# iSach/SoccerNeRFs

Measured on AMD Instinct MI355X. Metric: train rays/sec (K-Planes Broadcast-style, whole job), higher is better.
Workload: dtype bf16; 1 GPU; K-Planes default multiscale-res 1-16 on synthetic Broadcast-style (k-planes preset: 4096 rays/GPU/step, samples 256/128/64, 5 scales x 6 planes C=32, 156.0 M params), full train step incl. Adam; rays_per_gpu=4096, images=627, params=156049664, parallelism=single GPU

## Files before the change

### include/snerf.h

```cpp
#ifndef SNERF_H
#define SNERF_H

#include <stdint.h>

#ifdef __cplusplus
extern "C" {
#endif

typedef void* snerf_stream_t;

#define SNERF_OK 0
#define SNERF_ERR_ARG (-1)
#define SNERF_ERR_UNSUPPORTED (-2)

#define SNERF_MAX_SCALES 8
#define SNERF_ABI_VERSION 16
#define SNERF_ABI_REVISION 2

int snerf_abi_version(void);
int snerf_abi_revision(void);
const char* snerf_last_error(void);
const char* snerf_target_arch(void);

typedef struct {
// ... 177 lines not shown
  float* acc_out;
  float* depth_median;
  float* sqerr_rays;
  float* dist_rays;
  float* g_rgb;
  float* g_density;
  float* g_weights;
  int32_t* nonfinite_flag;
} snerf_ray_train_args;
int snerf_ray_train_fwd_bwd(const snerf_ray_train_args* args, snerf_stream_t stream);

int snerf_render_bwd(const float* weights, const float* rgb, const float* bg, int32_t bg_mode, const float* g_rgb_out,
                     const float* g_acc, int32_t R, int32_t S, float* g_weights, float* g_rgb, int32_t accumulate_w,
                     snerf_stream_t stream);

int snerf_render_mse_bwd(const float* weights, const float* rgb, const float* bg, int32_t bg_mode, const float* rgb_out, const float* target,
                         float go_scale, int32_t R, int32_t S, float* g_weights, float* g_rgb, float* sqerr_rays, snerf_stream_t stream);

int snerf_distortion(const float* weights, const float* sbins, int32_t R, int32_t S, float grad_scale, float* loss_rays,
                     float* g_weights, int32_t accumulate, snerf_stream_t stream);

int snerf_interlevel(const float* c_bins, const float* w_nerf, int32_t S, const float* p_bins, const float* w_prop, int32_t Sp,
                     int32_t R, float grad_scale, float* loss_rays, float* g_wprop, snerf_stream_t stream);

int snerf_depth_loss(const float* weights, const float* ebins, const float* termination_depth, const float* directions_norm, float sigma,
                     int32_t R, int32_t S, float grad_scale, float* loss_rays, float* g_weights, int32_t accumulate, snerf_stream_t stream);

int snerf_urf_depth_loss(const float* weights, const float* ebins, const float* termination_depth, const float* directions_norm,
                         const float* predicted_depth, float sigma, int32_t R, int32_t S, float grad_scale, float* loss_rays, float* g_weights,
                         float* g_predicted_depth, int32_t accumulate, snerf_stream_t stream);


int snerf_plane_reg(const snerf_kplanes_desc* desc, const float* planes, float* grad, float c_space_tv, float c_time_smooth,
                    float c_sparse, float* losses, int32_t n_slots, int32_t overwrite, snerf_stream_t stream);

typedef struct {
  int32_t nonfinite;
  int32_t t;
  int32_t skipped;
  int32_t dropped;
  float step_size;
  float inv_sqrt_bc2;
  int32_t skip;
  int32_t _pad;
} snerf_adam_dyn;
int snerf_adam_prepare(snerf_adam_dyn* dyn, float lr, float beta1, float beta2, int32_t policy, int32_t force_nonfinite, snerf_stream_t stream);
// ... 352 lines not shown
```

### soccernerfs_amd/_lib.py

```python
import ctypes as C
import os

import torch

_PKG = os.path.dirname(os.path.abspath(__file__))
LIB_PATH = os.path.join(_PKG, "libsnerf.so")

MAX_SCALES = 8
ABI_VERSION = 16
ABI_REVISION = 2


class KPlanesDesc(C.Structure):
    _c_struct_ = "snerf_kplanes_desc"
    _fields_ = [
        ("n_scales", C.c_int32),
        ("C", C.c_int32),
        ("concat", C.c_int32),
        ("n_coords", C.c_int32),
        ("res", (C.c_int32 * 4) * MAX_SCALES),
        ("off", (C.c_int64 * 6) * MAX_SCALES),
    ]


# ... 38 lines not shown
                ("gdens", C.c_void_p), ("grad_planes", C.c_void_p), ("workspace", C.c_void_p), ("gX", C.c_void_p)]


class AdamDyn(C.Structure):
    _c_struct_ = "snerf_adam_dyn"
    _fields_ = [("nonfinite", C.c_int32), ("t", C.c_int32), ("skipped", C.c_int32), ("dropped", C.c_int32),
                ("step_size", C.c_float), ("inv_sqrt_bc2", C.c_float), ("skip", C.c_int32), ("_pad", C.c_int32)]


class RenderArgs(C.Structure):
    _c_struct_ = "snerf_render_args"
    _fields_ = [("weights", C.c_void_p), ("rgb", C.c_void_p), ("ebins", C.c_void_p), ("bg", C.c_void_p),
                ("R", C.c_int32), ("S", C.c_int32), ("bg_mode", C.c_int32), ("training", C.c_int32),
                ("rgb_out", C.c_void_p), ("acc_out", C.c_void_p), ("depth_median", C.c_void_p), ("depth_expected", C.c_void_p),
                ("median_rgb", C.c_void_p), ("median_index", C.c_void_p)]


class RayTrainArgs(C.Structure):
    _c_struct_ = "snerf_ray_train_args"
    _fields_ = [("density", C.c_void_p), ("ebins", C.c_void_p), ("sbins", C.c_void_p), ("rgb", C.c_void_p), ("bg", C.c_void_p), ("target", C.c_void_p),
                ("R", C.c_int32), ("S", C.c_int32), ("bg_mode", C.c_int32), ("go_scale", C.c_float), ("dist_scale", C.c_float),
                ("weights", C.c_void_p), ("rgb_out", C.c_void_p), ("acc_out", C.c_void_p), ("depth_median", C.c_void_p), ("sqerr_rays", C.c_void_p),
                ("dist_rays", C.c_void_p), ("g_rgb", C.c_void_p), ("g_density", C.c_void_p), ("g_weights", C.c_void_p), ("nonfinite_flag", C.c_void_p)]


class RaygenArgs(C.Structure):
    _c_struct_ = "snerf_raygen_args"
    _fields_ = [("indices", C.c_void_p), ("fx", C.c_void_p), ("fy", C.c_void_p), ("cx", C.c_void_p), ("cy", C.c_void_p),
                ("c2w", C.c_void_p), ("cam_times", C.c_void_p),
                ("R", C.c_int32), ("collide", C.c_int32), ("training", C.c_int32), ("near_plane", C.c_float),
                ("aabb_min", C.c_float * 3), ("aabb_max", C.c_float * 3),
                ("origins", C.c_void_p), ("dirs", C.c_void_p), ("pixel_area", C.c_void_p), ("dir_norm", C.c_void_p),
                ("times", C.c_void_p), ("nears", C.c_void_p), ("fars", C.c_void_p)]


class RaygenFrameArgs(C.Structure):
    _c_struct_ = "snerf_raygen_frame_args"
    _fields_ = [("fx", C.c_float), ("fy", C.c_float), ("cx", C.c_float), ("cy", C.c_float), ("c2w", C.c_float * 12), ("time", C.c_float),
                ("W", C.c_int32), ("H", C.c_int32), ("_pad", C.c_int32), ("p0", C.c_int64), ("p1", C.c_int64),
                ("near_plane", C.c_float), ("aabb_min", C.c_float * 3), ("aabb_max", C.c_float * 3),
                ("origins", C.c_void_p), ("dirs", C.c_void_p), ("pixel_area", C.c_void_p), ("dir_norm", C.c_void_p),
                ("times", C.c_void_p), ("nears", C.c_void_p), ("fars", C.c_void_p)]


class RaygenLensArgs(C.Structure):
    _c_struct_ = "snerf_raygen_lens_args"
# ... 81 lines not shown
    "snerf_mlp_bwd_x16_quotient": "s:PPPILPIIPPIPIPPPP",
    "snerf_mlp_bwd_fx": "s:PPPILPIIPPIPP",
    "snerf_kplanes_field_fwd_supported": "i:PPP",
    "snerf_kplanes_field_fwd": "s:PPPLPPPPPPPPPP",
    "snerf_kplanes_field_fwd_ordered": "s:PPPLPPPPPPPPPPP",
    "snerf_kplanes_field_render_supported": "i:PPPI",
    "snerf_kplanes_field_render": "s:PPPIPPPPFPPPPPPP",
    "snerf_kplanes_color_input_fwd": "s:PIPLPP",
    "snerf_kplanes_color_input_bwd": "s:PILPP",
    "snerf_kplanes_color_bwd_vd_supported": "i:P",
    "snerf_kplanes_color_bwd_vd": "s:PPPIPLPIPPP",
    "snerf_kplanes_color_bwd_vd_ws": "s:PPPIPLPIPPP",
    "snerf_kplanes_density_fwd_supported": "i:PP",
    "snerf_kplanes_density_fwd": "s:PPPLPPPPP",
    "snerf_kplanes_density_bwd_supported": "i:PP",
    "snerf_kplanes_density_bwd": "s:PIP",
    "snerf_kplanes_density_bwd_budget": "s:PIIP",
    "snerf_render_fwd": "s:PP",
    "snerf_ray_train_fwd_bwd": "s:PP",
    "snerf_render_bwd": "s:PPPIPPIIPPIP",
    "snerf_render_mse_bwd": "s:PPPIPPFIIPPPP",
    "snerf_distortion": "s:PPIIFPPIP",
    "snerf_interlevel": "s:PPIPPIIFPPP",
    "snerf_depth_loss": "s:PPPPFIIFPPIP",
    "snerf_urf_depth_loss": "s:PPPPPFIIFPPPIP",
    "snerf_plane_reg": "s:PPPFFFPIIP",
    "snerf_adam_prepare": "s:PFFFIIP",
    "snerf_adam_step": "s:PPPPPLFFFFIFIPP",
    "snerf_adam_planes_step": "s:PPPPPPFFFPIFFFFIFIPP",
    "snerf_adam_planes_step_range": "s:PPPPPPFFFPIFFFFIFILLPP",
    "snerf_comm_unique_id": "s:P",
    "snerf_comm_create": "s:IIPP",
    "snerf_comm_destroy": "s:P",
    "snerf_allreduce_grads": "s:PPLP",
    "snerf_raygen": "s:PP",
    "snerf_raygen_frame": "s:PP",
    "snerf_raygen_lens": "s:PP",
    "snerf_raygen_frame_lens": "s:PP",
    "snerf_raygen_cam": "s:PP",
    "snerf_raygen_frame_cam": "s:PP",
    "snerf_pose_apply": "s:PPPIIPP",
    "snerf_raygen_pose_bwd": "s:PP",
    "snerf_sample_pixels_uniform": "s:PIIIIPPPP",
    "snerf_sample_pixels_sphere": "s:PIIIIPPPP",
    "snerf_mask_pack": "s:PLLLPPP",
    "snerf_sample_pixels_masked": "s:PIIIIPPLPPPP",
# ... 109 lines not shown
```

### soccernerfs_amd/csrc/per_ray_common.hpp

```cpp
#pragma once
#include "common.hpp"

namespace snerf {

constexpr int RAYS_PER_BLOCK = 4;
constexpr int MAX_S = 64 * WSCAN_PER;

struct BlockSync { __device__ __forceinline__ static void sync() { __syncthreads(); } };
struct WaveSync { __device__ __forceinline__ static void sync() { wave_lds_publish(); } };

template <typename Sync>
__device__ __forceinline__ void ray_optical_depth(const float* eb, const float* sigma, int n_sigma, float* dd, float* aux, int S, int lane) {
#pragma clang fp contract(off)
  for (int i = lane; i < S; i += 64) {
    const float e0 = eb[i], e1 = eb[i + 1];
    dd[i] = (e1 - e0) * (i < n_sigma ? sigma[i] : 0.f);
  }
  Sync::sync();
  wave_scan_f64<true, false>(dd, aux, S, lane);
  Sync::sync();
}

template <typename Sync>
__device__ __forceinline__ void ray_weights(const float* eb, const float* sigma, int n_sigma, float* dd, float* aux, float* w, float* w_out, bool live,
// ... 132 lines not shown
#pragma unroll
  for (int k = 0; k < WSCAN_PER; ++k) {
    const int i = lane + 64 * k;
    if (i < S) aux[i] = gwterm[k];
  }
  Sync::sync();
  wave_scan_f64<true, true>(aux, aux, S, lane);
  Sync::sync();
#pragma unroll
  for (int k = 0; k < WSCAN_PER; ++k) {
    const int i = lane + 64 * k;
    if (i < S && live) {
      const float g = gw[i];
      const float e0 = eb[i], e1 = eb[i + 1];
      const float gdd = g * Tk[k] * ek[k] - aux[i];
      float out = gdd * (e1 - e0);
      if (!(fabsf(out) <= 3.402823466e+38f)) { out = 0.f; bad = true; }
      if (accumulate) gdens[i] += out; else gdens[i] = out;
    }
  }
  return bad;
}

}
```

### soccernerfs_amd/csrc/raygen.hip

```cpp
#include "raygen_common.hpp"

#pragma clang fp contract(off)

namespace snerf {

struct RaygenArgs {
  const int64_t* indices;
  const float* fx; const float* fy; const float* cx; const float* cy;
  const float* c2w;
  const float* cam_times;
  int R;
  float* origins; float* dirs; float* pixel_area; float* dir_norm; float* times;
  int collide; int training; float near_plane;
  float aabb_min[3], aabb_max[3];
  float* nears; float* fars;
};

__global__ void raygen_kernel(RaygenArgs a) {
  int r = blockIdx.x * blockDim.x + threadIdx.x;
  if (r >= a.R) return;
  const int64_t c = a.indices[(int64_t)r * 3], yi = a.indices[(int64_t)r * 3 + 1], xi = a.indices[(int64_t)r * 3 + 2];
  const PixelRay p = pixel_ray(yi, xi, a.fx[c], a.fy[c], a.cx[c], a.cy[c], a.c2w + c * 12);
#pragma unroll
  for (int k = 0; k < 3; ++k) { a.origins[(int64_t)r * 3 + k] = p.o[k]; a.dirs[(int64_t)r * 3 + k] = p.d[k]; }
// ... 87 lines not shown
                                                        float* __restrict__ aux_out) {
  extern __shared__ uint32_t s_w[];
  for (int i = threadIdx.x; i < n_pow2; i += blockDim.x)
    s_w[i] = i < R ? (((uint32_t)image_key[idx_in[(int64_t)i * 3]] << 14) | (uint32_t)i) : 0xffffffffu;
  __syncthreads();
  for (int k = 2; k <= n_pow2; k <<= 1)
    for (int j = k >> 1; j > 0; j >>= 1) {
      for (int t = threadIdx.x; t < n_pow2 / 2; t += blockDim.x) {
        const int i = ((t / j) * 2 * j) + (t % j), l = i + j;
        const bool up = (i & k) == 0;
        const uint32_t a = s_w[i], b = s_w[l];
        if ((a > b) == up) { s_w[i] = b; s_w[l] = a; }
      }
      __syncthreads();
    }
  for (int r = threadIdx.x; r < R; r += blockDim.x) {
    const int64_t src = s_w[r] & 0x3fffu;
#pragma unroll
    for (int c = 0; c < 3; ++c) idx_out[(int64_t)r * 3 + c] = idx_in[src * 3 + c];
    for (int c = 0; c < aux_cols; ++c) aux_out[(int64_t)r * aux_cols + c] = aux_in[src * aux_cols + c];
  }
}

__global__ __launch_bounds__(256) void ray_time_order_kernel(const float* __restrict__ times, int R, int n_pow2, int32_t* __restrict__ order_out) {
  extern __shared__ uint64_t s_tk[];
  for (int i = threadIdx.x; i < n_pow2; i += blockDim.x)
    s_tk[i] = i < R ? (((uint64_t)__float_as_uint(times[i]) << 32) | (uint32_t)i) : ~0ull;
  __syncthreads();
  for (int k = 2; k <= n_pow2; k <<= 1)
    for (int lj = 31 - __clz(k >> 1); lj >= 0; --lj) {
      const int j = 1 << lj;
      for (int t = threadIdx.x; t < n_pow2 / 2; t += blockDim.x) {
        const int i = ((t >> lj) << (lj + 1)) | (t & (j - 1)), l = i + j;
        const bool up = (i & k) == 0;
        const uint64_t a = s_tk[i], b = s_tk[l];
        if ((a > b) == up) { s_tk[i] = b; s_tk[l] = a; }
      }
      __syncthreads();
    }
  for (int r = threadIdx.x; r < R; r += blockDim.x) order_out[r] = (int32_t)(uint32_t)s_tk[r];
}

__global__ void aabb_kernel(const float* __restrict__ o, const float* __restrict__ d, int R, float near_plane, int training, const float* amin3,
                            float* __restrict__ nears, float* __restrict__ fars, float a0, float a1, float a2, float b0, float b1, float b2) {
  int r = blockIdx.x * blockDim.x + threadIdx.x;
  if (r >= R) return;
  const float mn[3] = {a0, a1, a2}, mx[3] = {b0, b1, b2};
  float tn = -INFINITY, tf = INFINITY;
#pragma unroll
  for (int k = 0; k < 3; ++k) {
    float inv = 1.f / (d[(int64_t)r * 3 + k] + 1e-6f);
    float t1 = (mn[k] - o[(int64_t)r * 3 + k]) * inv, t2 = (mx[k] - o[(int64_t)r * 3 + k]) * inv;
    tn = fmaxf(tn, fminf(t1, t2));
    tf = fminf(tf, fmaxf(t1, t2));
  }
  tn = fmaxf(tn, training ? near_plane : 0.f);
  tf = fmaxf(tf, tn + 1e-6f);
  nears[r] = tn; fars[r] = tf;
}

__global__ void pose_apply_kernel(const float* __restrict__ c2w, const float* __restrict__ adj, const int32_t* __restrict__ group, int M, int G,
                                  float* __restrict__ out) {
  const int m = blockIdx.x * blockDim.x + threadIdx.x;
// ... 199 lines not shown
  if (R == 0) return 0;
  SNERF_REQUIRE(u && indices && (!images || target), "sample_pixels_uniform: null buffer");
  hipLaunchKernelGGL(sample_pixels_kernel, dim3(ceil_div(R, 256)), dim3(256), 0, (hipStream_t)stream, u, R, M, H, W, images, indices, target);
  SNERF_LAUNCH_CHECK("sample_pixels_uniform");
  return 0;
}

extern "C" int snerf_sort_rays_by_key(const int64_t* indices_in, const int32_t* image_key, int32_t n_keys, int32_t R, const float* aux_in,
                                      int32_t aux_cols, int64_t* indices_out, float* aux_out, snerf_stream_t stream) {
  SNERF_REQUIRE(R >= 0 && R <= 16384 && n_keys >= 1 && n_keys <= (1 << 18) && aux_cols >= 0,
                "sort_rays_by_key: R=%d (<= 16384) n_keys=%d (<= 262144) aux_cols=%d", R, n_keys, aux_cols);
  if (R == 0) return 0;
  SNERF_REQUIRE(indices_in && image_key && indices_out && indices_in != indices_out && (aux_cols == 0 || (aux_in && aux_out && aux_in != aux_out)),
                "sort_rays_by_key: null or aliased buffer (the sort is out of place)");
  int n = 2;
  while (n < R) n <<= 1;
  hipLaunchKernelGGL(sort_rays_kernel, dim3(1), dim3(256), (size_t)n * sizeof(uint32_t), (hipStream_t)stream, indices_in, image_key, R, n, aux_in, aux_cols,
                     indices_out, aux_out);
  SNERF_LAUNCH_CHECK("sort_rays_by_key");
  return 0;
}

extern "C" int snerf_ray_time_order(const float* times, int32_t R, int32_t* order_out, snerf_stream_t stream) {
  SNERF_REQUIRE(R >= 0 && R <= 16384, "ray_time_order: R=%d (<= 16384: one workgroup sorts in LDS)", R);
  if (R == 0) return 0;
  SNERF_REQUIRE(times && order_out, "ray_time_order: null buffer");
  int n = 2;
  while (n < R) n <<= 1;
  SNERF_ALLOW_LDS(ray_time_order_kernel, 16384 * (int)sizeof(uint64_t));
  hipLaunchKernelGGL(ray_time_order_kernel, dim3(1), dim3(256), (size_t)n * sizeof(uint64_t), (hipStream_t)stream, times, R, n, order_out);
  SNERF_LAUNCH_CHECK("ray_time_order");
  return 0;
}

extern "C" int snerf_aabb_collide(const float* origins, const float* dirs, int32_t R, const float* aabb6, float near_plane, int32_t training,
                                  float* nears, float* fars, snerf_stream_t stream) {
  SNERF_REQUIRE(R >= 0 && aabb6, "aabb_collide: bad arguments");
  if (R == 0) return 0;
  SNERF_REQUIRE(origins && dirs && nears && fars, "aabb_collide: null buffer");
  hipLaunchKernelGGL(aabb_kernel, dim3(ceil_div(R, 256)), dim3(256), 0, (hipStream_t)stream, origins, dirs, R, near_plane, training, nullptr, nears,
                     fars, aabb6[0], aabb6[1], aabb6[2], aabb6[3], aabb6[4], aabb6[5]);
  SNERF_LAUNCH_CHECK("aabb_collide");
  return 0;
}

extern "C" int snerf_pose_apply(const float* c2w, const float* pose_adjustment, const int32_t* group, int32_t M, int32_t G, float* c2w_adj,
                                snerf_stream_t stream) {
  SNERF_REQUIRE(M >= 0 && G >= 0, "pose_apply: M=%d G=%d", M, G);
  SNERF_REQUIRE(group || G == M, "pose_apply: no group table, so G=%d must equal M=%d", G, M);
  if (M == 0) return 0;
  SNERF_REQUIRE(c2w && pose_adjustment && c2w_adj, "pose_apply: null buffer");
  hipLaunchKernelGGL(pose_apply_kernel, dim3(ceil_div(M, 256)), dim3(256), 0, (hipStream_t)stream, c2w, pose_adjustment, group, M, G, c2w_adj);
  SNERF_LAUNCH_CHECK("pose_apply");
// ... 26 lines not shown
```

### soccernerfs_amd/csrc/render_loss.hip

```cpp
#include "per_ray_common.hpp"

#pragma clang fp contract(off)

namespace snerf {

struct RenderArgs {
  const float* weights;
  const float* rgb;
  const float* ebins;
  const float* bg;
  int R, S, bg_mode, training;
  float* rgb_out;
  float* acc_out;
  float* depth_median;
  float* depth_expected;
  float* median_rgb;
  int64_t* median_index;
};

__global__ __launch_bounds__(256) void render_fwd_kernel(RenderArgs a) {
  __shared__ float s_w[RAYS_PER_BLOCK][MAX_S];
  __shared__ float s_cum[RAYS_PER_BLOCK][MAX_S];
  __shared__ int s_med[RAYS_PER_BLOCK];
  const int wv = threadIdx.x >> 6, lane = threadIdx.x & 63;
// ... 64 lines not shown
  __shared__ float s_m[RAYS_PER_BLOCK][MAX_S];
  const int wv = threadIdx.x >> 6, lane = threadIdx.x & 63;
  const int ray = blockIdx.x * RAYS_PER_BLOCK + wv;
  const bool live = ray < R;
  const int r = live ? ray : R - 1;
  for (int i = lane; i < S; i += 64) s_w[wv][i] = weights[(int64_t)r * S + i];
  const float total = ray_distortion<BlockSync>(s_w[wv], s_m[wv], sbins + (int64_t)r * (S + 1), grad_scale,
                                                g_weights && live ? g_weights + (int64_t)r * S : nullptr, accumulate != 0, S, lane);
  if (lane == 0 && live && loss_rays) loss_rays[r] = total;
}

__global__ __launch_bounds__(256) void interlevel_kernel(const float* __restrict__ c_bins, const float* __restrict__ w_nerf, int S,
                                                        const float* __restrict__ p_bins, const float* __restrict__ w_prop, int Sp, int R,
                                                        float grad_scale, float* __restrict__ loss_rays, float* __restrict__ g_wprop) {
  __shared__ float s_tp[RAYS_PER_BLOCK][MAX_S + 1];
  __shared__ float s_cy[RAYS_PER_BLOCK][MAX_S + 1];
  __shared__ float s_g[RAYS_PER_BLOCK][MAX_S];
  __shared__ int s_lo[RAYS_PER_BLOCK][MAX_S];
  __shared__ int s_hi[RAYS_PER_BLOCK][MAX_S];
  const int wv = threadIdx.x >> 6, lane = threadIdx.x & 63;
  const int ray = blockIdx.x * RAYS_PER_BLOCK + wv;
  const bool live = ray < R;
  const int r = live ? ray : R - 1;
  float* tp = s_tp[wv];
  float* cy = s_cy[wv];
  for (int i = lane; i <= Sp; i += 64) tp[i] = p_bins[(int64_t)r * (Sp + 1) + i];
  for (int i = lane; i < Sp; i += 64) cy[i + 1] = w_prop[(int64_t)r * Sp + i];
  __syncthreads();
  wave_scan_f64<false, false>(cy + 1, cy + 1, Sp, lane);
  if (lane == 0) cy[0] = 0.f;
  __syncthreads();
  float total = 0.f;
  for (int i = lane; i < S; i += 64) {
    const float c0 = c_bins[(int64_t)r * (S + 1) + i], c1 = c_bins[(int64_t)r * (S + 1) + i + 1];
    int lo = 0, hi = Sp;
    while (lo < hi) { int mid = (lo + hi) >> 1; if (tp[mid] <= c0) lo = mid + 1; else hi = mid; }
    int ilo = lo - 1; ilo = ilo < 0 ? 0 : (ilo > Sp - 1 ? Sp - 1 : ilo);
    lo = 0; hi = Sp;
    while (lo < hi) { int mid = (lo + hi) >> 1; if (tp[mid + 1] <= c1) lo = mid + 1; else hi = mid; }
    int ihi = lo; ihi = ihi < 0 ? 0 : (ihi > Sp - 1 ? Sp - 1 : ihi);
    const float wo = cy[ihi + 1] - cy[ilo];
    const float w = w_nerf[(int64_t)r * S + i];
    const float d = fmaxf(w - wo, 0.f);
    total += d * d / (w + 1.0e-7f);
    s_lo[wv][i] = ilo; s_hi[wv][i] = ihi;
    s_g[wv][i] = -2.f * d / (w + 1.0e-7f);
  }
  total = wave_sum(total);
  if (lane == 0 && live && loss_rays) loss_rays[r] = total;
  __syncthreads();
  if (g_wprop) {
    const int* slo = s_lo[wv];
    const int* shi = s_hi[wv];
    for (int j = lane; j < Sp; j += 64) {
      int a = 0, e = S;
      while (a < e) { const int mid = (a + e) >> 1; if (shi[mid] < j) a = mid + 1; else e = mid; }
      int b = 0;
      e = S;
      while (b < e) { const int mid = (b + e) >> 1; if (slo[mid] <= j) b = mid + 1; else e = mid; }
      float acc = 0.f;
      for (int i = a; i < b; ++i) acc += s_g[wv][i];
      if (live) g_wprop[(int64_t)r * Sp + j] = acc * grad_scale;
    }
  }
}

__global__ __launch_bounds__(256) void depth_loss_kernel(const float* __restrict__ weights, const float* __restrict__ ebins, const float* __restrict__ term,
                                                        const float* __restrict__ dir_norm, float sigma, int R, int S, float grad_scale,
                                                        float* __restrict__ loss_rays, float* __restrict__ g_weights, int accumulate) {
  const int wv = threadIdx.x >> 6, lane = threadIdx.x & 63;
  const int ray = blockIdx.x * RAYS_PER_BLOCK + wv;
  if (ray >= R) return;
  float D = term[ray];
  if (dir_norm) D = D * dir_norm[ray];
  const bool on = D > 0.f;
  float total = 0.f;
  for (int i = lane; i < S; i += 64) {
    const float e0 = ebins[(int64_t)ray * (S + 1) + i], e1 = ebins[(int64_t)ray * (S + 1) + i + 1];
    const float w = weights[(int64_t)ray * S + i];
    const float t = (e0 + e1) / 2.f;
    const float k = expf(-((t - D) * (t - D)) / (2.f * sigma)) * (e1 - e0);
    total += -logf(w + 1.0e-7f) * k;
    if (g_weights) {
      const float g = on ? grad_scale * (-k / (w + 1.0e-7f)) : 0.f;
      if (accumulate) g_weights[(int64_t)ray * S + i] += g; else g_weights[(int64_t)ray * S + i] = g;
    }
  }
// ... 169 lines not shown

extern "C" int snerf_distortion(const float* weights, const float* sbins, int32_t R, int32_t S, float grad_scale, float* loss_rays,
                                float* g_weights, int32_t accumulate, snerf_stream_t stream) {
  SNERF_REQUIRE(R >= 0 && S >= 1 && S <= MAX_S, "distortion: R=%d S=%d (S <= %d)", R, S, MAX_S);
  if (R == 0) return 0;
  SNERF_REQUIRE(weights && sbins, "distortion: null buffer");
  hipLaunchKernelGGL(distortion_kernel, dim3(ceil_div(R, RAYS_PER_BLOCK)), dim3(256), 0, (hipStream_t)stream, weights, sbins, R, S, grad_scale, loss_rays,
                     g_weights, accumulate);
  SNERF_LAUNCH_CHECK("distortion");
  return 0;
}

extern "C" int snerf_interlevel(const float* c_bins, const float* w_nerf, int32_t S, const float* p_bins, const float* w_prop, int32_t Sp,
                                int32_t R, float grad_scale, float* loss_rays, float* g_wprop, snerf_stream_t stream) {
  SNERF_REQUIRE(R >= 0 && S >= 1 && S <= MAX_S && Sp >= 1 && Sp <= MAX_S, "interlevel: R=%d S=%d Sp=%d", R, S, Sp);
  if (R == 0) return 0;
  SNERF_REQUIRE(c_bins && w_nerf && p_bins && w_prop, "interlevel: null buffer");
  hipLaunchKernelGGL(interlevel_kernel, dim3(ceil_div(R, RAYS_PER_BLOCK)), dim3(256), 0, (hipStream_t)stream, c_bins, w_nerf, S, p_bins, w_prop, Sp, R,
                     grad_scale, loss_rays, g_wprop);
  SNERF_LAUNCH_CHECK("interlevel");
  return 0;
}

extern "C" int snerf_ray_train_fwd_bwd(const snerf_ray_train_args* p, snerf_stream_t stream) {
  SNERF_REQUIRE(p, "ray_train_fwd_bwd: null args");
  SNERF_REQUIRE(p->R >= 0 && p->S >= 1 && p->S <= MAX_S, "ray_train_fwd_bwd: R=%d S=%d (S <= %d)", p->R, p->S, MAX_S);
  SNERF_REQUIRE(p->bg_mode == 0 || p->bg_mode == 2, "ray_train_fwd_bwd: bg_mode %d has no training backward", p->bg_mode);
  if (p->R == 0) return 0;
  SNERF_REQUIRE(p->density && p->ebins && p->sbins && p->rgb && p->bg && p->target && p->weights && p->rgb_out && p->acc_out && p->g_rgb && p->g_density,
                "ray_train_fwd_bwd: null buffer");
  RayTrainArgs a = {};
  a.density = p->density; a.ebins = p->ebins; a.sbins = p->sbins; a.rgb = p->rgb; a.bg = p->bg; a.target = p->target;
  a.R = p->R; a.S = p->S; a.bg_mode = p->bg_mode; a.go_scale = p->go_scale; a.dist_scale = p->dist_scale;
  a.weights = p->weights; a.rgb_out = p->rgb_out; a.acc_out = p->acc_out; a.depth_median = p->depth_median; a.sqerr_rays = p->sqerr_rays;
  a.dist_rays = p->dist_rays; a.g_rgb = p->g_rgb; a.g_density = p->g_density; a.g_weights = p->g_weights; a.nonfinite_flag = p->nonfinite_flag;
  hipLaunchKernelGGL(ray_train_kernel, dim3(ceil_div(p->R, RAYS_PER_BLOCK)), dim3(256), 0, (hipStream_t)stream, a);
  SNERF_LAUNCH_CHECK("ray_train_fwd_bwd");
  return 0;
}
```

### soccernerfs_amd/fused_step.py

```python
import ctypes as C
import math
from typing import Dict, Optional, Sequence, Tuple

import torch

from . import _lib


def anneal_value(step: int, max_iters: int, slope: float) -> float:
    frac = min(max(step / max_iters, 0.0), 1.0)
    return (slope * frac) / ((slope - 1) * frac + 1)


def update_schedule(step: int, warmup: int, every: int) -> float:
    return min(max(every * min(max(step / warmup, 0.0), 1.0), 1.0), float(every))


def cosine_lr_factor(step: int, warm_up_end: int, max_steps: int, alpha: float) -> float:
    if step < warm_up_end:
        return step / warm_up_end
    progress = (step - warm_up_end) / (max_steps - warm_up_end)
    return (math.cos(math.pi * progress) + 1.0) * 0.5 * (1 - alpha) + alpha


# ... 156 lines not shown
        ra.weights, ra.rgb_out, ra.acc_out = b["w"][2].data_ptr(), b["rgb_out"].data_ptr(), b["acc"].data_ptr()
        ra.depth_median = b["depth"].data_ptr() if median_depth else None
        ra.sqerr_rays, ra.dist_rays, ra.g_rgb, ra.g_density = b["sqerr"].data_ptr(), b["dist_rays"].data_ptr(), b["grgb"].data_ptr(), b["gdens"][2].data_ptr()
        ra.g_weights, ra.nonfinite_flag = None, dyn.data_ptr() if dyn is not None else None
        with self._span("ray_train_fwd_bwd"):
            self._call("ray_train_fwd_bwd", C.byref(ra), self._st)

    def _mse_distortion_bwd(self, target, bg, go_scale: float, dist_scale: float):
        b, R, S2 = self.buf, self.R, self.S[2]
        self._call("render_mse_bwd", self._p(b["w"][2]), self._p(b["rgb"]), self._p(bg), 0, self._p(b["rgb_out"]), self._p(target), go_scale, R, S2,
                   self._p(b["gw"][2]), self._p(b["grgb"]), self._p(b["sqerr"]), self._st)
        self._call("distortion", self._p(b["w"][2]), self._p(b["sb"][2]), R, S2, dist_scale, self._p(b["dist_rays"]), self._p(b["gw"][2]), 1,
                   self._st)

    def _weights_bwd(self, lvl: int, dyn: Optional[torch.Tensor] = None):
        b = self.buf
        self._call("weights_bwd", self._p(b["dens"][lvl]), self._p(b["eb"][lvl]), self._p(b["gw"][lvl]), self.R, self.S[lvl], self._p(b["gdens"][lvl]),
                   0, self._p(dyn) if dyn is not None else None, self._st)

    def _interlevel(self, lvl: int, mult: float, with_grad: bool):
        b, R, S2 = self.buf, self.R, self.S[2]
        self._call("interlevel", self._p(b["sb"][2]), self._p(b["w"][2]), S2, self._p(b["sb"][lvl]), self._p(b["w"][lvl]), self.S[lvl], R,
                   mult / (R * S2), self._p(b["inter_rays"][lvl]), self._p(b["gw"][lvl]) if with_grad else None, self._st)
```

### soccernerfs_amd/trainer.py

```python
import ctypes as C
from dataclasses import dataclass, field
from typing import Dict, List, Optional, Sequence, Tuple

import torch

from . import _lib, ops
from .fused_step import FusedStep, _On, _align4, anneal_value, cosine_lr_factor, update_schedule
from .streams import side_stream
from .plane_set import PlaneSet
from .tcnn_compat import Network


@dataclass
class KPlanesTrainConfig:

    aabb_scale: float = 1.5
    spacetime_resolution: Sequence[int] = (64, 64, 64, 100)
    multiscale_res: Sequence[int] = (1, 2, 4, 8, 16)
    feature_dim: int = 32
    proposal_resolutions: Sequence[Sequence[int]] = ((128, 128, 128, 100), (256, 256, 256, 100))
    proposal_feature_dim: int = 8
    sigma_net_hidden_dim: int = 128
    rgb_net_hidden_dim: int = 64
    disable_viewing_dependent: bool = True
# ... 25 lines not shown
    proposal_operands: Optional[str] = None
    gvec_dtype: str = "fp32"
    overlap: bool = True
    async_field_adam: bool = True
    defer_prop: bool = True
    fused_ray_loss: bool = True
    sorted_scatter: bool = True
    fuse_reg_into_adam: bool = True
    shard_optimizer: bool = True
    mlp_grad_workspace: bool = True
    interleave_proposal_levels: bool = False
    fix_capacity: Optional[int] = None
    exchange_chunks: int = 2
    grad_transport: str = "fp32"
    param_transport: str = "fp32"
    emulate_transports: str = ""
    deterministic: bool = False
    nonfinite_policy: str = "skip_step"
    fused_field: bool = True
    quotient_scatter: bool = True
    quotient_epilogue: bool = True
    fused_proposal: bool = True
    fused_proposal_backward: bool = True
    proposal_backward_workgroups_per_cu: float = 1.0
    pass_b_beside_head: bool = True
    sort_before_field_fwd: bool = False
    field_fwd_time_order: bool = True
    pipeline_sweep: str = ""
    ray_gradients: bool = False
    freeze_time_planes: bool = False
    freeze_space_planes: bool = False


class KPlanesTrainer(FusedStep):

    def __init__(self, cfg: KPlanesTrainConfig, num_rays: int, device="cuda:0", process_group=None):
        self.cfg, self.R, self.dev = cfg, num_rays, torch.device(device)
        self.pg = process_group
        self.world = torch.distributed.get_world_size(process_group) if process_group is not None else 1
        self.rank = torch.distributed.get_rank(process_group) if process_group is not None else 0
        nc = len(cfg.spacetime_resolution)
        if nc not in (3, 4) or any(len(r) != nc for r in cfg.proposal_resolutions):
            raise ValueError(f"spacetime_resolution and every entry of proposal_resolutions must all have 3 (static scene) or all have 4 values; got "
                             f"{list(cfg.spacetime_resolution)} and {[list(r) for r in cfg.proposal_resolutions]}")
        if cfg.freeze_time_planes and nc == 3:
            raise ValueError("freeze_time_planes on a 3-coordinate model (len(spacetime_resolution) == 3): it has no time planes to freeze")
# ... 477 lines not shown
                if not passb_issued:
                    main = torch.cuda.current_stream()
                    st = self._stream("adam")
                    st.wait_stream(main)
                    with _On(self, st):
                        self._scatter_field_scales(co, 0, ns, fixup=False)
                    self._passb_done = st.record_event()
            else:
                self._scatter_field_scales(co, 0, ns)
        else:
            self._scatter(self._desc_field, self.field_planes.planes, co, N, sl(b["gfeat"]), self.gviews["field.planes"])

    def _depth_loss(self, lvl: int, with_grad: bool):
        if self._depth is None:
            return
        cfg, b, R = self.cfg, self.buf, self.R
        dn = None if cfg.is_euclidean_depth else self.rays["directions_norm"]
        self._call("depth_loss", self._p(b["w"][lvl]), self._p(b["eb"][lvl]), self._p(self._depth), self._p(dn) if dn is not None else None,
                   cfg.depth_sigma, R, self.S[lvl], cfg.loss_coefficients["depth_loss"] / (3 * R), self._p(b["depth_rays"][lvl]),
                   self._p(b["gw"][lvl]) if with_grad else None, 1, self._st)

    def _proposal_backward(self, proposal_grads: bool):
        cfg, b, R, co = self.cfg, self.buf, self.R, self.cfg.loss_coefficients
        for lvl in (0, 1):
            self._interlevel(lvl, co["interlevel_loss"], proposal_grads)
            self._depth_loss(lvl, with_grad=proposal_grads)
        if not proposal_grads:
            return
        wb = lambda lvl: self._weights_bwd(lvl, self._dyn["proposal_networks"])
        nb = lambda lvl: self._mlp_bwd(self.prop_nets[lvl], f"prop{lvl}.mlp", b["pfeat"][lvl], cfg.proposal_feature_dim, R * self.S[lvl], None, 1, 0,
                                       b["gdens"][lvl], b["gpfeat"][lvl], cfg.proposal_feature_dim)
        sc = lambda lvl: self._scatter(self._desc_prop[lvl], self.prop_planes[lvl].planes, self._coords[lvl], R * self.S[lvl], b["gpfeat"][lvl],
                                       self.gviews[f"prop{lvl}.planes"])
        if self.fused_proposal_backward:
            for lvl in (0, 1):
                wb(lvl)
            self._fused_proposal_backward()
        elif cfg.interleave_proposal_levels:
            for stage in (wb, nb, sc):
                for lvl in (0, 1):
                    stage(lvl)
        else:
            for lvl in (0, 1):
                for stage in (wb, nb, sc):
                    stage(lvl)
        if cfg.ray_gradients:
            for lvl in (0, 1):
                self._ray_gradient(self._desc_prop[lvl], self.prop_planes[lvl].planes, self._coords[lvl], R * self.S[lvl], b["gpfeat"][lvl])

    def _fused_proposal_backward(self):
        cfg, b, R = self.cfg, self.buf, self.R
        levels = (_lib.DensityBwdLevel * 2)()
        for lvl in (0, 1):
            L, net = levels[lvl], self.prop_nets[lvl]
            L.desc, L.planes, L.coords = C.addressof(self._desc_prop[lvl]), self.prop_planes[lvl].planes.data_ptr(), C.addressof(self._coords[lvl])
            L.N, L.net, L.W, L.gdens = R * self.S[lvl], C.addressof(net.desc), net.params.data_ptr(), b["gdens"][lvl].data_ptr()
            L.grad_planes, L.workspace = self.gviews[f"prop{lvl}.planes"].data_ptr(), self._mlp_ws[f"prop{lvl}.mlp"].data_ptr()
            L.gX = b["gpfeat"][lvl].data_ptr() if cfg.ray_gradients else None
            self._ws_dirty.add(f"prop{lvl}.mlp")
# ... 512 lines not shown
```

Baseline: 2.141 million rays/s.

## Parallelize ray time ordering via rank counting and add fused proposal ray backward

Replaces the single-workgroup bitonic sort of ray times with a multi-workgroup rank-count kernel: each group of 16 lanes counts how many keys are smaller than its ray's key and scatters the ray index to that rank. Also adds an optional kernel that fuses the interlevel loss and proposal weights backward for both proposal levels into one launch, sharing a refactored device helper. The fused path is off by default; the sort change does O(R^2) comparisons but spreads them over many CUs instead of one workgroup.

```diff
diff --git a/include/snerf.h b/include/snerf.h
--- a/include/snerf.h
+++ b/include/snerf.h
@@ -223,6 +223,20 @@
 
 int snerf_interlevel(const float* c_bins, const float* w_nerf, int32_t S, const float* p_bins, const float* w_prop, int32_t Sp,
                      int32_t R, float grad_scale, float* loss_rays, float* g_wprop, snerf_stream_t stream);
+
+typedef struct {
+  const float* p_bins;
+  const float* w_prop;
+  const float* density;
+  const float* ebins;
+  float* loss_rays;
+  float* g_density;
+  float* g_weights;
+  int32_t Sp;
+  float grad_scale;
+} snerf_proposal_ray_level;
+int snerf_proposal_ray_bwd(const float* c_bins, const float* w_nerf, int32_t S, const snerf_proposal_ray_level* levels, int32_t n_levels,
+                           int32_t R, int32_t with_grad, int32_t* nonfinite_flag, snerf_stream_t stream);
 
 int snerf_depth_loss(const float* weights, const float* ebins, const float* termination_depth, const float* directions_norm, float sigma,
                      int32_t R, int32_t S, float grad_scale, float* loss_rays, float* g_weights, int32_t accumulate, snerf_stream_t stream);
diff --git a/soccernerfs_amd/_lib.py b/soccernerfs_amd/_lib.py
--- a/soccernerfs_amd/_lib.py
+++ b/soccernerfs_amd/_lib.py
@@ -84,6 +84,12 @@
                 ("R", C.c_int32), ("S", C.c_int32), ("bg_mode", C.c_int32), ("go_scale", C.c_float), ("dist_scale", C.c_float),
                 ("weights", C.c_void_p), ("rgb_out", C.c_void_p), ("acc_out", C.c_void_p), ("depth_median", C.c_void_p), ("sqerr_rays", C.c_void_p),
                 ("dist_rays", C.c_void_p), ("g_rgb", C.c_void_p), ("g_density", C.c_void_p), ("g_weights", C.c_void_p), ("nonfinite_flag", C.c_void_p)]
+
+
+class ProposalRayLevel(C.Structure):
+    _c_struct_ = "snerf_proposal_ray_level"
+    _fields_ = [("p_bins", C.c_void_p), ("w_prop", C.c_void_p), ("density", C.c_void_p), ("ebins", C.c_void_p), ("loss_rays", C.c_void_p),
+                ("g_density", C.c_void_p), ("g_weights", C.c_void_p), ("Sp", C.c_int32), ("grad_scale", C.c_float)]
 
 
 class RaygenArgs(C.Structure):
@@ -211,6 +217,7 @@
     "snerf_render_mse_bwd": "s:PPPIPPFIIPPPP",
     "snerf_distortion": "s:PPIIFPPIP",
     "snerf_interlevel": "s:PPIPPIIFPPP",
+    "snerf_proposal_ray_bwd": "s:PPIPIIIPP",
     "snerf_depth_loss": "s:PPPPFIIFPPIP",
     "snerf_urf_depth_loss": "s:PPPPPFIIFPPPIP",
     "snerf_plane_reg": "s:PPPFFFPIIP",
diff --git a/soccernerfs_amd/csrc/per_ray_common.hpp b/soccernerfs_amd/csrc/per_ray_common.hpp
--- a/soccernerfs_amd/csrc/per_ray_common.hpp
+++ b/soccernerfs_amd/csrc/per_ray_common.hpp
@@ -178,4 +178,50 @@
   return bad;
 }
 
-}
+template <typename Sync>
+__device__ __forceinline__ float ray_interlevel(const float* c_bins, const float* w_nerf, int S, const float* p_bins, const float* w_prop, int Sp, float* tp,
+                                                float* cy, float* g, int* lo_row, int* hi_row, float grad_scale, float* gw_row, float* gw_out, bool live,
+                                                int lane) {
+#pragma clang fp contract(off)
+  for (int i = lane; i <= Sp; i += 64) tp[i] = p_bins[i];
+  for (int i = lane; i < Sp; i += 64) cy[i + 1] = w_prop[i];
+  Sync::sync();
+  wave_scan_f64<false, false>(cy + 1, cy + 1, Sp, lane);
+  if (lane == 0) cy[0] = 0.f;
+  Sync::sync();
+  float total = 0.f;
+  for (int i = lane; i < S; i += 64) {
+    const float c0 = c_bins[i], c1 = c_bins[i + 1];
+    int lo = 0, hi = Sp;
+    while (lo < hi) { int mid = (lo + hi) >> 1; if (tp[mid] <= c0) lo = mid + 1; else hi = mid; }
+    int ilo = lo - 1; ilo = ilo < 0 ? 0 : (ilo > Sp - 1 ? Sp - 1 : ilo);
+    lo = 0; hi = Sp;
+    while (lo < hi) { int mid = (lo + hi) >> 1; if (tp[mid + 1] <= c1) lo = mid + 1; else hi = mid; }
+    int ihi = lo; ihi = ihi < 0 ? 0 : (ihi > Sp - 1 ? Sp - 1 : ihi);
+    const float wo = cy[ihi + 1] - cy[ilo];
+    const float w = w_nerf[i];
+    const float d = fmaxf(w - wo, 0.f);
+    total += d * d / (w + 1.0e-7f);
+    lo_row[i] = ilo; hi_row[i] = ihi;
+    g[i] = -2.f * d / (w + 1.0e-7f);
+  }
+  total = wave_sum(total);
+  Sync::sync();
+  if (gw_row || gw_out) {
+    for (int j = lane; j < Sp; j += 64) {
+      int a = 0, e = S;
+      while (a < e) { const int mid = (a + e) >> 1; if (hi_row[mid] < j) a = mid + 1; else e = mid; }
+      int b = 0;
+      e = S;
+      while (b < e) { const int mid = (b + e) >> 1; if (lo_row[mid] <= j) b = mid + 1; else e = mid; }
+      float acc = 0.f;
+      for (int i = a; i < b; ++i) acc += g[i];
+      const float gv = acc * grad_scale;
+      if (gw_row) gw_row[j] = gv;
+      if (gw_out && live) gw_out[j] = gv;
+    }
+  }
+  return total;
+}
+
+}
diff --git a/soccernerfs_amd/csrc/raygen.hip b/soccernerfs_amd/csrc/raygen.hip
--- a/soccernerfs_amd/csrc/raygen.hip
+++ b/soccernerfs_amd/csrc/raygen.hip
@@ -133,23 +133,25 @@
   }
 }
 
-__global__ __launch_bounds__(256) void ray_time_order_kernel(const float* __restrict__ times, int R, int n_pow2, int32_t* __restrict__ order_out) {
-  extern __shared__ uint64_t s_tk[];
-  for (int i = threadIdx.x; i < n_pow2; i += blockDim.x)
-    s_tk[i] = i < R ? (((uint64_t)__float_as_uint(times[i]) << 32) | (uint32_t)i) : ~0ull;
+constexpr int kTimeOrderRays = 16;
+__global__ __launch_bounds__(256) void ray_time_order_kernel(const float* __restrict__ times, int R, int n_pad, int32_t* __restrict__ order_out) {
+  extern __shared__ uint4 s_t4[];
+  uint32_t* s_t = reinterpret_cast<uint32_t*>(s_t4);
+  for (int i = threadIdx.x; i < n_pad; i += blockDim.x) s_t[i] = i < R ? __float_as_uint(times[i]) : 0xffffffffu;
   __syncthreads();
-  for (int k = 2; k <= n_pow2; k <<= 1)
-    for (int lj = 31 - __clz(k >> 1); lj >= 0; --lj) {
-      const int j = 1 << lj;
-      for (int t = threadIdx.x; t < n_pow2 / 2; t += blockDim.x) {
-        const int i = ((t >> lj) << (lj + 1)) | (t & (j - 1)), l = i + j;
-        const bool up = (i & k) == 0;
-        const uint64_t a = s_tk[i], b = s_tk[l];
-        if ((a > b) == up) { s_tk[i] = b; s_tk[l] = a; }
-      }
-      __syncthreads();
-    }
-  for (int r = threadIdx.x; r < R; r += blockDim.x) order_out[r] = (int32_t)(uint32_t)s_tk[r];
+  const int sub = threadIdx.x & 15, ray = blockIdx.x * kTimeOrderRays + (threadIdx.x >> 4);
+  const bool live = ray < R;
+  const uint64_t mine = ((uint64_t)(live ? s_t[ray] : 0u) << 32) | (uint32_t)ray;
+  int below = 0;
+  for (int q = sub; q < n_pad / 4; q += 16) {
+    const uint4 w = s_t4[q];
+    const uint32_t j = (uint32_t)q * 4u;
+    below += (int)((((uint64_t)w.x << 32) | j) < mine) + (int)((((uint64_t)w.y << 32) | (j + 1u)) < mine) +
+             (int)((((uint64_t)w.z << 32) | (j + 2u)) < mine) + (int)((((uint64_t)w.w << 32) | (j + 3u)) < mine);
+  }
+#pragma unroll
+  for (int off = 8; off > 0; off >>= 1) below += __shfl_xor(below, off, 64);
+  if (live && sub == 0) order_out[below] = ray;
 }
 
 __global__ void aabb_kernel(const float* __restrict__ o, const float* __restrict__ d, int R, float near_plane, int training, const float* amin3,
@@ -395,13 +397,12 @@
 }
 
 extern "C" int snerf_ray_time_order(const float* times, int32_t R, int32_t* order_out, snerf_stream_t stream) {
-  SNERF_REQUIRE(R >= 0 && R <= 16384, "ray_time_order: R=%d (<= 16384: one workgroup sorts in LDS)", R);
+  SNERF_REQUIRE(R >= 0 && R <= 16384, "ray_time_order: R=%d (<= 16384: every workgroup holds the R time words in 64 KB of LDS)", R);
   if (R == 0) return 0;
   SNERF_REQUIRE(times && order_out, "ray_time_order: null buffer");
-  int n = 2;
-  while (n < R) n <<= 1;
-  SNERF_ALLOW_LDS(ray_time_order_kernel, 16384 * (int)sizeof(uint64_t));
-  hipLaunchKernelGGL(ray_time_order_kernel, dim3(1), dim3(256), (size_t)n * sizeof(uint64_t), (hipStream_t)stream, times, R, n, order_out);
+  const int n_pad = ceil_div(R, 64) * 64;
+  hipLaunchKernelGGL(ray_time_order_kernel, dim3(ceil_div(R, kTimeOrderRays)), dim3(256), (size_t)n_pad * sizeof(uint32_t), (hipStream_t)stream, times, R,
+                     n_pad, order_out);
   SNERF_LAUNCH_CHECK("ray_time_order");
   return 0;
 }
diff --git a/soccernerfs_amd/csrc/render_loss.hip b/soccernerfs_amd/csrc/render_loss.hip
--- a/soccernerfs_amd/csrc/render_loss.hip
+++ b/soccernerfs_amd/csrc/render_loss.hip
@@ -110,47 +110,53 @@
   const int ray = blockIdx.x * RAYS_PER_BLOCK + wv;
   const bool live = ray < R;
   const int r = live ? ray : R - 1;
-  float* tp = s_tp[wv];
-  float* cy = s_cy[wv];
-  for (int i = lane; i <= Sp; i += 64) tp[i] = p_bins[(int64_t)r * (Sp + 1) + i];
-  for (int i = lane; i < Sp; i += 64) cy[i + 1] = w_prop[(int64_t)r * Sp + i];
+  const float total = ray_interlevel<BlockSync>(c_bins + (int64_t)r * (S + 1), w_nerf + (int64_t)r * S, S, p_bins + (int64_t)r * (Sp + 1),
+                                                w_prop + (int64_t)r * Sp, Sp, s_tp[wv], s_cy[wv], s_g[wv], s_lo[wv], s_hi[wv], grad_scale, nullptr,
+                                                g_wprop ? g_wprop + (int64_t)r * Sp : nullptr, live, lane);
+  if (lane == 0 && live && loss_rays) loss_rays[r] = total;
+}
+
+constexpr int PROP_RAY_MAX_LEVELS = 4;
+struct PropRayLevel {
+  const float* p_bins; const float* w_prop; const float* density; const float* ebins;
+  float* loss_rays; float* g_density; float* g_weights;
+  int Sp; float grad_scale;
+};
+struct PropRayArgs {
+  const float* c_bins; const float* w_nerf;
+  int S, R, blocks_per_level, with_grad;
+  int32_t* nonfinite_flag;
+  PropRayLevel lv[PROP_RAY_MAX_LEVELS];
+};
+
+__global__ __launch_bounds__(256) void proposal_ray_bwd_kernel(PropRayArgs a) {
+  __shared__ float s_tp[RAYS_PER_BLOCK][MAX_S + 1];
+  __shared__ float s_cy[RAYS_PER_BLOCK][MAX_S + 1];
+  __shared__ float s_g[RAYS_PER_BLOCK][MAX_S];
+  __shared__ int s_lo[RAYS_PER_BLOCK][MAX_S];
+  __shared__ int s_hi[RAYS_PER_BLOCK][MAX_S];
+  __shared__ float s_gw[RAYS_PER_BLOCK][MAX_S];
+  const int wv = __builtin_amdgcn_readfirstlane(threadIdx.x >> 6), lane = threadIdx.x & 63;
+  const int lvl = blockIdx.x / a.blocks_per_level;
+  const int ray = (blockIdx.x - lvl * a.blocks_per_level) * RAYS_PER_BLOCK + wv;
+  PropRayLevel L = a.lv[0];
+#pragma unroll
+  for (int k = 1; k < PROP_RAY_MAX_LEVELS; ++k)
+    if (lvl == k) L = a.lv[k];
+  const bool live = ray < a.R;
+  const int r = live ? ray : a.R - 1;
+  const int S = a.S, Sp = L.Sp;
+  const bool grad = a.with_grad != 0;
+  const float total = ray_interlevel<BlockSync>(a.c_bins + (int64_t)r * (S + 1), a.w_nerf + (int64_t)r * S, S, L.p_bins + (int64_t)r * (Sp + 1),
+                                                L.w_prop + (int64_t)r * Sp, Sp, s_tp[wv], s_cy[wv], s_g[wv], s_lo[wv], s_hi[wv], L.grad_scale,
+                                                grad ? s_gw[wv] : nullptr, grad && L.g_weights ? L.g_weights + (int64_t)r * Sp : nullptr, live, lane);
+  if (lane == 0 && live && L.loss_rays) L.loss_rays[r] = total;
+  if (!grad) return;
   __syncthreads();
-  wave_scan_f64<false, false>(cy + 1, cy + 1, Sp, lane);
-  if (lane == 0) cy[0] = 0.f;
-  __syncthreads();
-  float total = 0.f;
-  for (int i = lane; i < S; i += 64) {
-    const float c0 = c_bins[(int64_t)r * (S + 1) + i], c1 = c_bins[(int64_t)r * (S + 1) + i + 1];
-    int lo = 0, hi = Sp;
-    while (lo < hi) { int mid = (lo + hi) >> 1; if (tp[mid] <= c0) lo = mid + 1; else hi = mid; }
-    int ilo = lo - 1; ilo = ilo < 0 ? 0 : (ilo > Sp - 1 ? Sp - 1 : ilo);
-    lo = 0; hi = Sp;
-    while (lo < hi) { int mid = (lo + hi) >> 1; if (tp[mid + 1] <= c1) lo = mid + 1; else hi = mid; }
-    int ihi = lo; ihi = ihi < 0 ? 0 : (ihi > Sp - 1 ? Sp - 1 : ihi);
-    const float wo = cy[ihi + 1] - cy[ilo];
-    const float w = w_nerf[(int64_t)r * S + i];
-    const float d = fmaxf(w - wo, 0.f);
-    total += d * d / (w + 1.0e-7f);
-    s_lo[wv][i] = ilo; s_hi[wv][i] = ihi;
-    s_g[wv][i] = -2.f * d / (w + 1.0e-7f);
-  }
-  total = wave_sum(total);
-  if (lane == 0 && live && loss_rays) loss_rays[r] = total;
-  __syncthreads();
-  if (g_wprop) {
-    const int* slo = s_lo[wv];
-    const int* shi = s_hi[wv];
-    for (int j = lane; j < Sp; j += 64) {
-      int a = 0, e = S;
-      while (a < e) { const int mid = (a + e) >> 1; if (shi[mid] < j) a = mid + 1; else e = mid; }
-      int b = 0;
-      e = S;
-      while (b < e) { const int mid = (b + e) >> 1; if (slo[mid] <= j) b = mid + 1; else e = mid; }
-      float acc = 0.f;
-      for (int i = a; i < b; ++i) acc += s_g[wv][i];
-      if (live) g_wprop[(int64_t)r * Sp + j] = acc * grad_scale;
-    }
-  }
+  const float* eb = L.ebins + (int64_t)r * (Sp + 1);
+  ray_optical_depth<BlockSync>(eb, L.density + (int64_t)r * Sp, Sp, s_tp[wv], s_cy[wv], Sp, lane);
+  const bool bad = ray_weights_bwd<BlockSync>(s_tp[wv], s_cy[wv], s_gw[wv], eb, L.g_density + (int64_t)r * Sp, false, live, Sp, lane);
+  if (bad && a.nonfinite_flag) *a.nonfinite_flag = 1;
 }
 
 __global__ __launch_bounds__(256) void depth_loss_kernel(const float* __restrict__ weights, const float* __restrict__ ebins, const float* __restrict__ term,
@@ -366,6 +372,28 @@
   return 0;
 }
 
+extern "C" int snerf_proposal_ray_bwd(const float* c_bins, const float* w_nerf, int32_t S, const snerf_proposal_ray_level* levels, int32_t n_levels,
+                                      int32_t R, int32_t with_grad, int32_t* nonfinite_flag, snerf_stream_t stream) {
+  SNERF_REQUIRE(R >= 0 && S >= 1 && S <= MAX_S && n_levels >= 1 && n_levels <= PROP_RAY_MAX_LEVELS && levels,
+                "proposal_ray_bwd: R=%d S=%d (S <= %d) n_levels=%d (1..%d)", R, S, MAX_S, n_levels, PROP_RAY_MAX_LEVELS);
+  PropRayArgs a = {};
+  for (int l = 0; l < n_levels; ++l) {
+    const snerf_proposal_ray_level& p = levels[l];
+    SNERF_REQUIRE(p.Sp >= 1 && p.Sp <= MAX_S, "proposal_ray_bwd: level %d Sp=%d (1..%d)", l, p.Sp, MAX_S);
+    SNERF_REQUIRE(R == 0 || (p.p_bins && p.w_prop && (!with_grad || (p.density && p.ebins && p.g_density))), "proposal_ray_bwd: level %d: null buffer", l);
+    PropRayLevel& L = a.lv[l];
+    L.p_bins = p.p_bins; L.w_prop = p.w_prop; L.density = p.density; L.ebins = p.ebins; L.loss_rays = p.loss_rays; L.g_density = p.g_density;
+    L.g_weights = p.g_weights; L.Sp = p.Sp; L.grad_scale = p.grad_scale;
+  }
+  if (R == 0) return 0;
+  SNERF_REQUIRE(c_bins && w_nerf, "proposal_ray_bwd: null buffer");
+  a.c_bins = c_bins; a.w_nerf = w_nerf; a.S = S; a.R = R; a.blocks_per_level = ceil_div(R, RAYS_PER_BLOCK); a.with_grad = with_grad != 0;
+  a.nonfinite_flag = nonfinite_flag;
+  hipLaunchKernelGGL(proposal_ray_bwd_kernel, dim3(a.blocks_per_level * n_levels), dim3(256), 0, (hipStream_t)stream, a);
+  SNERF_LAUNCH_CHECK("proposal_ray_bwd");
+  return 0;
+}
+
 extern "C" int snerf_ray_train_fwd_bwd(const snerf_ray_train_args* p, snerf_stream_t stream) {
   SNERF_REQUIRE(p, "ray_train_fwd_bwd: null args");
   SNERF_REQUIRE(p->R >= 0 && p->S >= 1 && p->S <= MAX_S, "ray_train_fwd_bwd: R=%d S=%d (S <= %d)", p->R, p->S, MAX_S);
diff --git a/soccernerfs_amd/fused_step.py b/soccernerfs_amd/fused_step.py
--- a/soccernerfs_amd/fused_step.py
+++ b/soccernerfs_amd/fused_step.py
@@ -202,3 +202,15 @@
         b, R, S2 = self.buf, self.R, self.S[2]
         self._call("interlevel", self._p(b["sb"][2]), self._p(b["w"][2]), S2, self._p(b["sb"][lvl]), self._p(b["w"][lvl]), self.S[lvl], R,
                    mult / (R * S2), self._p(b["inter_rays"][lvl]), self._p(b["gw"][lvl]) if with_grad else None, self._st)
+
+    def _proposal_ray_bwd(self, mult: float, with_grad: bool, dyn: Optional[torch.Tensor] = None):
+        b, R, S2 = self.buf, self.R, self.S[2]
+        levels = (_lib.ProposalRayLevel * 2)()
+        for lvl in (0, 1):
+            L = levels[lvl]
+            L.p_bins, L.w_prop, L.density, L.ebins = b["sb"][lvl].data_ptr(), b["w"][lvl].data_ptr(), b["dens"][lvl].data_ptr(), b["eb"][lvl].data_ptr()
+            L.loss_rays, L.g_density, L.g_weights = b["inter_rays"][lvl].data_ptr(), b["gdens"][lvl].data_ptr(), None
+            L.Sp, L.grad_scale = self.S[lvl], mult / (R * S2)
+        with self._span("proposal_ray_bwd"):
+            self._call("proposal_ray_bwd", self._p(b["sb"][2]), self._p(b["w"][2]), S2, levels, 2, R, int(with_grad),
+                       self._p(dyn) if dyn is not None and with_grad else None, self._st)
diff --git a/soccernerfs_amd/trainer.py b/soccernerfs_amd/trainer.py
--- a/soccernerfs_amd/trainer.py
+++ b/soccernerfs_amd/trainer.py
@@ -71,6 +71,7 @@
     quotient_epilogue: bool = True
     fused_proposal: bool = True
     fused_proposal_backward: bool = True
+    fused_proposal_ray_bwd: bool = False
     proposal_backward_workgroups_per_cu: float = 1.0
     pass_b_beside_head: bool = True
     sort_before_field_fwd: bool = False
@@ -594,19 +595,26 @@
 
     def _proposal_backward(self, proposal_grads: bool):
         cfg, b, R, co = self.cfg, self.buf, self.R, self.cfg.loss_coefficients
-        for lvl in (0, 1):
-            self._interlevel(lvl, co["interlevel_loss"], proposal_grads)
-            self._depth_loss(lvl, with_grad=proposal_grads)
+        one_launch = cfg.fused_proposal_ray_bwd and self._depth is None
+        if one_launch:
+            self._proposal_ray_bwd(co["interlevel_loss"], proposal_grads, self._dyn["proposal_networks"])
+        else:
+            with self._span("proposal_interlevel"):
+                for lvl in (0, 1):
+                    self._interlevel(lvl, co["interlevel_loss"], proposal_grads)
+                    self._depth_loss(lvl, with_grad=proposal_grads)
         if not proposal_grads:
             return
-        wb = lambda lvl: self._weights_bwd(lvl, self._dyn["proposal_networks"])
+        wb = (lambda lvl: None) if one_launch else (lambda lvl: self._weights_bwd(lvl, self._dyn["proposal_networks"]))
         nb = lambda lvl: self._mlp_bwd(self.prop_nets[lvl], f"prop{lvl}.mlp", b["pfeat"][lvl], cfg.proposal_feature_dim, R * self.S[lvl], None, 1, 0,
                                        b["gdens"][lvl], b["gpfeat"][lvl], cfg.proposal_feature_dim)
         sc = lambda lvl: self._scatter(self._desc_prop[lvl], self.prop_planes[lvl].planes, self._coords[lvl], R * self.S[lvl], b["gpfeat"][lvl],
                                        self.gviews[f"prop{lvl}.planes"])
         if self.fused_proposal_backward:
-            for lvl in (0, 1):
-                wb(lvl)
+            if not one_launch:
+                with self._span("proposal_weights_bwd"):
+                    for lvl in (0, 1):
+                        wb(lvl)
             self._fused_proposal_backward()
         elif cfg.interleave_proposal_levels:
             for stage in (wb, nb, sc):
```

New measurement: 2.126 million rays/s. Within noise of the previous version (-0.7%).
